# RegulatoryGenomicsGroup/chicdiff

Hardware: NVIDIA B200
Metric: regions tested/sec (agg+NB GLM+dispersion+Wald) (higher is better)
Workload: dtype f64

## Files before the change

chicdiff_b200/csrc/context.cu:

```cuda
#include "../../include/chicdiff_b200.h"
#include "kernels.h"
#include "comm.h"
#include "results_host.h"
#include <algorithm>
#include <climits>
#include <cmath>
#include <cstdarg>
#include <cstdio>
#include <cstdlib>
#include <cstring>
#include <string>
#include <vector>
#include <unistd.h>

using namespace cd;

namespace {

thread_local std::string g_create_error;

template <typename T> struct DevBuf {
    T* p = nullptr;
    size_t cap = 0;
    ~DevBuf() { if (p) cudaFree(p); }
// ... 25 lines not shown
        }
    }
    for (int i = 0; i < p; i++) for (int j = 0; j < p; j++) inv[i * p + j] = a[i][p + j];
    return true;
}

bool build_design(int S, int p, const double* X, CdDesign& d)
{
    memset(&d, 0, sizeof(d));
    d.S = S; d.p = p;
    for (int i = 0; i < S * p; i++) d.X[i] = X[i];
    double xtx[CD_MAXP * CD_MAXP], inv[CD_MAXP * CD_MAXP];
    for (int a = 0; a < p; a++)
        for (int b = 0; b < p; b++) {
            double s = 0;
            for (int j = 0; j < S; j++) s += X[j * p + a] * X[j * p + b];
            xtx[a * p + b] = s;
        }
    if (!invert_small(xtx, p, inv)) return false;
    for (int u = 0; u < p; u++)
        for (int j = 0; j < S; j++) {
            double s = 0;
            for (int v = 0; v < p; v++) s += inv[u * p + v] * X[j * p + v];
            d.ls[u * S + j] = s;
        }
    for (int a = 0; a < S; a++)
        for (int b = 0; b < S; b++) {
            double s = 0;
            for (int u = 0; u < p; u++) s += X[a * p + u] * d.ls[u * S + b];
            d.hat[a * S + b] = s;
        }
    d.ncell = 0;
    for (int j = 0; j < S; j++) {
        int found = -1;
        for (int k = 0; k < j && found < 0; k++) {
            bool same = true;
            for (int u = 0; u < p; u++) if (X[j * p + u] != X[k * p + u]) same = false;
            if (same) found = d.cell[k];
        }
        if (found < 0) { found = d.ncell++; d.cell_size[found] = 0; }
        d.cell[j] = found;
        d.cell_size[found]++;
    }
    d.linear_mu = (d.ncell == p);
    d.any3 = 0;
    for (int c = 0; c < d.ncell; c++) if (d.cell_size[c] >= 3) d.any3 = 1;
    return true;
}

double trigamma_host(double x)
{
    double r = 0.0;
    while (x < 10.0) { r += 1.0 / (x * x); x += 1.0; }
    const double f = 1.0 / (x * x);
    return r + 1.0 / x + 0.5 * f +
           (1.0 / x) * f * (1.0 / 6.0 + f * (-1.0 / 30.0 + f * (1.0 / 42.0 + f * (-1.0 / 30.0 +
           f * (5.0 / 66.0 + f * (-691.0 / 2730.0 + f * (7.0 / 6.0)))))));
}

__global__ void __launch_bounds__(256) dfma_peak_kernel(int iters, double m, double* __restrict__ sink)
{
    double a0 = threadIdx.x, a1 = a0 + 1, a2 = a0 + 2, a3 = a0 + 3, a4 = a0 + 4, a5 = a0 + 5, a6 = a0 + 6, a7 = a0 + 7;
    const double c = 1e-9;
#pragma unroll 16
    for (int k = 0; k < iters; k++) {
        a0 = fma(a0, m, c); a1 = fma(a1, m, c); a2 = fma(a2, m, c); a3 = fma(a3, m, c);
        a4 = fma(a4, m, c); a5 = fma(a5, m, c); a6 = fma(a6, m, c); a7 = fma(a7, m, c);
    }
    const double r = ((a0 + a1) + (a2 + a3)) + ((a4 + a5) + (a6 + a7));
    if (r == 123.456) *sink = r;
}

__global__ void count_evals_kernel(int64_t n, const int32_t* __restrict__ iter, unsigned long long* __restrict__ out)
{
    unsigned long long local = 0;
    for (int64_t i = (int64_t)blockIdx.x * blockDim.x + threadIdx.x; i < n; i += (int64_t)gridDim.x * blockDim.x) {
        const int it = iter[i];
        if (it > 0) local += (unsigned long long)it + 1ull;
    }
    for (int off = 16; off > 0; off >>= 1) local += __shfl_down_sync(0xffffffffu, local, off);
    if ((threadIdx.x & 31) == 0 && local) atomicAdd(out, local);
}

__global__ void count_flags_kernel(int64_t n, const uint8_t* __restrict__ flags, unsigned long long* __restrict__ out)
{
    const int64_t i = (int64_t)blockIdx.x * blockDim.x + threadIdx.x;
    const uint8_t f = (i < n) ? flags[i] : (uint8_t)CD_FLAG_ALLZERO;
    const unsigned nz = __ballot_sync(0xffffffffu, (i < n) && !(f & CD_FLAG_ALLZERO));
    const unsigned gg = __ballot_sync(0xffffffffu, (i < n) && (f & CD_FLAG_GENE_GRID));
    const unsigned mg = __ballot_sync(0xffffffffu, (i < n) && (f & CD_FLAG_MAP_GRID));
    const unsigned bn = __ballot_sync(0xffffffffu, (i < n) && (f & CD_FLAG_BETA_NOCONV));
    if ((threadIdx.x & 31) == 0) {
        if (nz) atomicAdd(out + 0, (unsigned long long)__popc(nz));
        if (gg) atomicAdd(out + 1, (unsigned long long)__popc(gg));
        if (mg) atomicAdd(out + 2, (unsigned long long)__popc(mg));
        if (bn) atomicAdd(out + 3, (unsigned long long)__popc(bn));
    }
}

constexpr int kScalSf = 0;
constexpr int kScalXim = 64;
constexpr int kScalMed = 96;
constexpr int kScalMad = 128;
constexpr int kScalDev = 160;
constexpr int kScalTrend = 192;
constexpr int kScalSums = 384;
constexpr int kScalSize = 1024;
constexpr int kPinTrend = 0, kPinMad = 128, kPinErr = 144, kPinBad = 145, kPinDev = 160, kPinTrendIn = 200, kPinSf = 400;

constexpr int kCntFlags = 0;
constexpr int kCntWait = 4;
constexpr int kCntBad = 7;
constexpr int kCntSelBar = 8;
constexpr int kCntTrendBar = 9;
constexpr int kCntErr = 10;
constexpr int kCntFitDispQueue = 12;
constexpr int kCntPark = 14;
constexpr int kCntWaldQueue = 15;
constexpr int kCntSize = 16;

}

struct cd_ctx {
    int device = 0;
    cudaStream_t st = nullptr;
    std::string err;
    int64_t launches = 0;
    double timings[8] = {0, 0, 0, 0, 0, 0, 0, 0};
    Comm comm;

    bool have_design = false;
    CdDesign des{}, des1{};
    DevBuf<CdDesign> des_dev;
    int64_t n = 0, R = 0;
    bool have_regions = false, have_agg = false, rows_borrowed = false;
    bool have_results = false;
    std::vector<uint8_t> sample_set;
    DevBuf<int64_t> row_off;
    DevBuf<int32_t> N_rows, N_rows_alt;
    DevBuf<double> FM_rows, FM_rows_alt;
    cudaStream_t st_copy = nullptr;
    cudaEvent_t ev_copy = nullptr;
    cudaEvent_t ev_tab_copy = nullptr, ev_tab_used = nullptr;
    bool tab_copy_pending = false;
    cudaEvent_t ev_read[2] = {nullptr, nullptr};
    int front = 0;
    bool front_used = false;
    std::vector<uint8_t> staged;
    int32_t* nbuf(int b) { return b ? N_rows_alt.p : N_rows.p; }
    double* fbuf(int b) { return b ? FM_rows_alt.p : FM_rows.p; }
    int back() const { return front_used ? 1 - front : front; }
    DevBuf<double> BM_rows;
    bool have_bm_rows = false;
    const int32_t* N_rows_p = nullptr;
    const double* FM_rows_p = nullptr;
    DevBuf<int32_t> K;
    DevBuf<double> FM;
    DevBuf<int32_t> Kb;
    int64_t batch_cap = 0;
    DevBuf<double> nf, mu, baseVar, rough, alpha_init, log_alpha, initial_lp, last_lp, dispMAP, dispersion,
        beta, betaSE, stat, pvalue, deviance, maxCooks;
    DevBuf<int32_t> dispGeneIter, dispIter, betaIter, refit_list;
    DevBuf<double> g_baseMean, g_dispGeneEst, g_dispFit, g_resid;
    DevBuf<uint8_t> g_flags;
    DevBuf<double> g_LR;
    DevBuf<unsigned long long> sel_state, sel_hist, sel_aux;
    DevBuf<double> trend_xs;
    DevBuf<double> start_log, log_fit;
    DevBuf<double> partial, scal;
    DevBuf<unsigned long long> counters;
    DevBuf<unsigned long long> eval_counts;
    int n_eval_calls = 0;
    int eval_call_p[16] = {0};
    int64_t eval_call_regions[16] = {0};
    unsigned long long eval_counts_host[16] = {0};
    double trend_passes_batch = 0;
    double trend_passes = 0;
    unsigned long long wait_host[3] = {0, 0, 0};
    DevBuf<int32_t> refit_count;
    DevBuf<int64_t> park_row;
// ... 1241 lines not shown
    CD_CUDA(ctx, ctx->dispGeneIter.ensure(vn)); CD_CUDA(ctx, ctx->dispIter.ensure(vn));
    CD_CUDA(ctx, ctx->betaIter.ensure((size_t)n)); CD_CUDA(ctx, ctx->refit_list.ensure(vn));
    CD_CUDA(ctx, ctx->g_baseMean.ensure(vn)); CD_CUDA(ctx, ctx->g_dispGeneEst.ensure(vn));
    CD_CUDA(ctx, ctx->g_dispFit.ensure(vn)); CD_CUDA(ctx, ctx->g_resid.ensure(vn));
    CD_CUDA(ctx, ctx->g_flags.ensure(vn)); CD_CUDA(ctx, ctx->trend_xs.ensure(vn));
    CD_CUDA(ctx, ctx->start_log.ensure(vn)); CD_CUDA(ctx, ctx->log_fit.ensure(vn));
    CD_CUDA(ctx, ctx->partial.ensure((size_t)kReduceBlocks * kMaxBatch * (CD_MAXS + 1)));
    CD_CUDA(ctx, ctx->scal.ensure(kScalSize));
    if (!ctx->counters.p) {
        CD_CUDA(ctx, ctx->counters.ensure(kCntSize));
        CD_CUDA(ctx, cudaMemsetAsync(ctx->counters.p, 0, kCntSize * sizeof(unsigned long long), st));
    }
    CD_CUDA(ctx, ctx->refit_count.ensure(1));
    CD_CUDA(ctx, ctx->wald_c.ensure((size_t)S * (size_t)n));
    CD_CUDA(ctx, ctx->wald_b0.ensure((size_t)CD_MAXP * (size_t)n));
    CD_CUDA(ctx, ctx->wald_b.ensure((size_t)CD_MAXP * (size_t)n));
    CD_CUDA(ctx, ctx->wald_iter.ensure((size_t)n));
    if (!ctx->lfact.p) {
        CD_CUDA(ctx, ctx->lfact.ensure(kLfactN));
        CD_LAUNCHN(ctx, 1, launch_lfact_table(ctx->lfact.p, st));
    }
    ctx->wald_ws.lfact = ctx->lfact.p;
    ctx->wald_ws.cmat = ctx->wald_c.p; ctx->wald_ws.beta0 = ctx->wald_b0.p; ctx->wald_ws.beta_nat = ctx->wald_b.p;
    ctx->wald_ws.iter = ctx->wald_iter.p; ctx->wald_ws.work_counter = ctx->counters.p + kCntWaldQueue;
    {
        const int64_t cap = nv / 4 + 4096;
        CD_CUDA(ctx, ctx->park_row.ensure((size_t)cap));
        CD_CUDA(ctx, ctx->park_d.ensure((size_t)cap * 5));
        CD_CUDA(ctx, ctx->park_i.ensure((size_t)cap * 2));
        FitDispPark& pk = ctx->park;
        pk.capacity = cap; pk.row = ctx->park_row.p;
        pk.a = ctx->park_d.p; pk.lp = pk.a + cap; pk.dlp = pk.lp + cap; pk.kappa = pk.dlp + cap; pk.lp0 = pk.kappa + cap;
        pk.iter = ctx->park_i.p; pk.iter_accept = pk.iter + cap;
        pk.count = ctx->counters.p + kCntPark;
    }

    CD_CUDA(ctx, ctx->eval_counts.ensure(16));
    CD_CUDA(ctx, cudaMemsetAsync(ctx->eval_counts.p, 0, 16 * sizeof(unsigned long long), st));
    CD_CUDA(ctx, cudaMemsetAsync(ctx->counters.p + kCntWait, 0, 4 * sizeof(unsigned long long), st));
    ctx->n_eval_calls = 0;
    ctx->trend_passes = 0;
    CD_CUDA(ctx, cudaEventRecord(ctx->ev[2], st));
    memset(out->sizeFactors, 0, sizeof(out->sizeFactors));
    for (int k = 2; k < 8; k++) ctx->timings[k] = 0.0;
    ctx->ev_used = 0;
    ctx->tm_begin(6);
    int rc = size_factors(ctx, out->sizeFactors);
    if (rc != CD_OK) return rc;
    ctx->tm_end();

    out->n_deviances = 0;
    BatchOut bo{};
    if (use_grid) {
        rc = run_batch(ctx, ctx->des1, ctx->des_dev.p + 1, ng, CD_NORM_COMBINED, grid, opt->disp_prior_var_grid, grid_len, false, bo, opt);
        if (rc != CD_OK) return rc;
        for (int k = 0; k < ng; k++) {
            out->deviances[k] = bo.sum_deviance[k];
            if (std::isnan(bo.sum_deviance[k]))
                return ctx->fail(CD_ENUMERIC, "theta grid: total deviance is NA (an all-zero region is present and chicdiff.R:1647 "
                                              "sums without na.rm); pass theta explicitly, as chicdiffPipeline does for the control set");
        }
        out->n_deviances = ng;
        int best = -1, nbest = 0;
        for (int k = 0; k < ng; k++) {
            if (best < 0 || out->deviances[k] < out->deviances[best]) { best = k; nbest = 1; }
            else if (out->deviances[k] == out->deviances[best]) nbest++;
        }
        if (nbest != 1) return ctx->fail(CD_ENUMERIC, "theta grid: the minimum total deviance is tied");
        theta = grid[best];
    }
    const double theta_final = std::isnan(theta) ? 0.0 : theta;
    rc = run_batch(ctx, ctx->des, ctx->des_dev.p, 1, norm, &theta_final, opt->disp_prior_var, grid_len, true, bo, opt);
    if (rc != CD_OK) return rc;
    CD_CUDA(ctx, cudaEventRecord(ctx->ev[3], st));
    struct { double a0, a1, varLogDispEsts, dispPriorVar; } po = {bo.a0[0], bo.a1[0], bo.varLogDispEsts[0], bo.dispPriorVar[0]};

    out->theta = (norm == CD_NORM_COMBINED) ? theta : NAN;
    out->trend_a0 = po.a0; out->trend_a1 = po.a1;
    out->varLogDispEsts = po.varLogDispEsts; out->dispPriorVar = po.dispPriorVar;

    CD_CUDA(ctx, cudaMemsetAsync(ctx->counters.p + kCntFlags, 0, 4 * sizeof(unsigned long long), st));
    const uint8_t* flags = ctx->g_flags.p + ctx->g_off;
    if (n > 0) {
        count_flags_kernel<<<(unsigned)((n + 255) / 256), 256, 0, st>>>(n, flags, ctx->counters.p + kCntFlags);
        ctx->launches++;
    }
    unsigned long long hc[4] = {0, 0, 0, 0};
    CD_CUDA(ctx, cudaMemcpyAsync(hc, ctx->counters.p + kCntFlags, sizeof(hc), cudaMemcpyDeviceToHost, st));
    CD_CUDA(ctx, cudaMemcpyAsync(ctx->eval_counts_host, ctx->eval_counts.p, sizeof(ctx->eval_counts_host), cudaMemcpyDeviceToHost, st));
    CD_CUDA(ctx, cudaMemcpyAsync(ctx->wait_host, ctx->counters.p + kCntWait, sizeof(ctx->wait_host), cudaMemcpyDeviceToHost, st));
    const size_t nn = (size_t)n;
    if ((rc = d2h(ctx, out->baseMean, ctx->g_baseMean.p + ctx->g_off, nn)) != CD_OK) return rc;
    if ((rc = d2h(ctx, out->baseVar, ctx->baseVar.p, nn)) != CD_OK) return rc;
    if ((rc = d2h(ctx, out->dispGeneEst, ctx->g_dispGeneEst.p + ctx->g_off, nn)) != CD_OK) return rc;
    if ((rc = d2h(ctx, out->dispFit, ctx->g_dispFit.p + ctx->g_off, nn)) != CD_OK) return rc;
    if ((rc = d2h(ctx, out->dispMAP, ctx->dispMAP.p, nn)) != CD_OK) return rc;
    if ((rc = d2h(ctx, out->dispersion, ctx->dispersion.p, nn)) != CD_OK) return rc;
    if ((rc = d2h(ctx, out->log2FoldChange, ctx->beta.p + (size_t)(p - 1) * nn, nn)) != CD_OK) return rc;
    if ((rc = d2h(ctx, out->lfcSE, ctx->betaSE.p + (size_t)(p - 1) * nn, nn)) != CD_OK) return rc;
    if ((rc = d2h(ctx, out->beta, ctx->beta.p, (size_t)p * nn)) != CD_OK) return rc;
    if ((rc = d2h(ctx, out->betaSE, ctx->betaSE.p, (size_t)p * nn)) != CD_OK) return rc;
    if ((rc = d2h(ctx, out->stat, ctx->stat.p, nn)) != CD_OK) return rc;
    if ((rc = d2h(ctx, out->pvalue, ctx->pvalue.p, nn)) != CD_OK) return rc;
    if ((rc = d2h(ctx, out->deviance, ctx->deviance.p, nn)) != CD_OK) return rc;
    if ((rc = d2h(ctx, out->maxCooks, ctx->maxCooks.p, nn)) != CD_OK) return rc;
    if ((rc = d2h(ctx, out->normFactors, ctx->nf.p, (size_t)S * nn)) != CD_OK) return rc;
    if ((rc = d2h(ctx, out->mu, ctx->mu.p, (size_t)S * nn)) != CD_OK) return rc;
    if ((rc = d2h(ctx, out->dispGeneIter, ctx->dispGeneIter.p, nn)) != CD_OK) return rc;
    if ((rc = d2h(ctx, out->dispIter, ctx->dispIter.p, nn)) != CD_OK) return rc;
    if ((rc = d2h(ctx, out->betaIter, ctx->betaIter.p, nn)) != CD_OK) return rc;
    if ((rc = d2h(ctx, out->flags, flags, nn)) != CD_OK) return rc;
    CD_CUDA(ctx, cudaStreamSynchronize(st));
    out->n_nonzero = (int64_t)hc[0]; out->n_gene_grid = (int64_t)hc[1];
    out->n_map_grid = (int64_t)hc[2]; out->n_beta_noconv = (int64_t)hc[3];
    float ms = 0;
    cudaEventElapsedTime(&ms, ctx->ev[2], ctx->ev[3]);
    ctx->timings[1] = ms;
    ctx->tm_collect();
    ctx->have_results = true;
    return CD_OK;
}

static int results_on_device(cd_ctx* ctx, int64_t n, int S, int p, const double* baseMean, const double* maxCooks,
                             const uint8_t* flags, const double* pvalue, double* pvalue_out, double* padj_out, double* scalars_out)
{
    cudaStream_t st = ctx->st;
    const double alpha = 0.1;
    const double cutoff = res_qf(0.99, (double)p, (double)(S - p));
    const size_t nn = (size_t)std::max<int64_t>(n, 1);
    const int C = res_chunks(n);
    for (int k = 0; k < 4; k++) CD_CUDA(ctx, ctx->res_key[k].ensure(nn));
    for (int k = 0; k < 2; k++) CD_CUDA(ctx, ctx->res_idx[k].ensure(nn));
    CD_CUDA(ctx, ctx->res_pv.ensure(nn)); CD_CUDA(ctx, ctx->res_padj.ensure(nn));
    CD_CUDA(ctx, ctx->res_bms.ensure(nn)); CD_CUDA(ctx, ctx->res_ps.ensure(nn));
    CD_CUDA(ctx, ctx->res_cnt.ensure((size_t)50 * (size_t)std::max(C, 1)));
    CD_CUDA(ctx, ctx->res_cmin.ensure((size_t)std::max(C, 1))); CD_CUDA(ctx, ctx->res_smin.ensure((size_t)std::max(C, 1)));
    CD_CUDA(ctx, ctx->res_small.ensure(2 + 50 + 50));
    CD_CUDA(ctx, ctx->res_smalld.ensure(100));
    unsigned long long* counts = ctx->res_small.p;
    unsigned long long* m_tot = ctx->res_small.p + 2;
    unsigned long long* best = ctx->res_small.p + 52;
    double* cut = ctx->res_smalld.p;
    double* theta = ctx->res_smalld.p + 50;
    unsigned long long *pkey0 = ctx->res_key[0].p, *pkey1 = ctx->res_key[1].p, *bmkey0 = ctx->res_key[2].p, *bmkey1 = ctx->res_key[3].p;
    unsigned int *idx0 = ctx->res_idx[0].p, *idx1 = ctx->res_idx[1].p;

    CD_LAUNCHN(ctx, 1, res_launch_keys(n, p, cutoff, baseMean, maxCooks, flags, pvalue, ctx->res_pv.p, ctx->res_padj.p,
                                       pkey0, bmkey0, idx0, counts, st));
    int j = 0;
    double cut_h[50], theta_h[50];
    for (int k = 0; k < 50; k++) { cut_h[k] = NAN; theta_h[k] = (k == 49) ? .95 : 0.0 + k * ((.95 - 0.0) / 49); }
    if (n > 0) {
        size_t bytes = 0;
        CD_CUDA(ctx, cp_sort_pairs_u64(nullptr, bytes, bmkey0, bmkey1, idx0, idx1, n, st));
        CD_CUDA(ctx, ctx->res_tmp.ensure(bytes));
        CD_LAUNCHN(ctx, 1, cp_sort_pairs_u64(ctx->res_tmp.p, bytes, bmkey0, bmkey1, idx0, idx1, n, st));
        CD_LAUNCHN(ctx, 1, res_launch_cutoffs(n, bmkey1, counts, cut, theta, st));
        CD_LAUNCHN(ctx, 1, cp_sort_pairs_u64(ctx->res_tmp.p, bytes, pkey0, pkey1, idx0, idx1, n, st));
        CD_LAUNCHN(ctx, 1, res_launch_gather(n, idx1, baseMean, ctx->res_pv.p, ctx->res_bms.p, ctx->res_ps.p, st));
        CD_LAUNCHN(ctx, 3, res_launch_num_rej(n, counts, ctx->res_bms.p, ctx->res_ps.p, cut, ctx->res_cnt.p, m_tot, alpha, best, st));
        unsigned long long best_h[50];
        CD_CUDA(ctx, cudaMemcpyAsync(best_h, best, sizeof(best_h), cudaMemcpyDeviceToHost, st));
        CD_CUDA(ctx, cudaMemcpyAsync(cut_h, cut, sizeof(cut_h), cudaMemcpyDeviceToHost, st));
        CD_CUDA(ctx, cudaMemcpyAsync(theta_h, theta, sizeof(theta_h), cudaMemcpyDeviceToHost, st));
        CD_CUDA(ctx, cudaStreamSynchronize(st));
        double numRej[50];
        for (int k = 0; k < 50; k++) numRej[k] = (double)best_h[k];
// ... 169 lines not shown
```

chicdiff_b200/csrc/dispersion.cu:

```cuda
#include "kernels.h"
#include <cuda_pipeline.h>
#include "posterior.cuh"

namespace cd {

static inline int blocks_for(int64_t n, int threads) { return (int)((n + threads - 1) / threads); }

__global__ void __launch_bounds__(256)
norm_factors_kernel(int64_t n, int S, int G, const double* __restrict__ FMagg, const double* __restrict__ sf,
                    int mode, BatchScalars theta, double* __restrict__ nf, const int32_t* __restrict__ K,
                    int32_t* __restrict__ Kb)
{
    const int64_t i = (int64_t)blockIdx.x * blockDim.x + threadIdx.x;
    if (i >= n) return;
    const int64_t nv = (int64_t)G * n;
    if (Kb) {
        for (int s = 0; s < S; s++) {
            const int32_t k = K[(int64_t)s * n + i];
            for (int g = 0; g < G; g++) Kb[(int64_t)s * nv + (int64_t)g * n + i] = k;
        }
    }
    if (mode == 0) {
        for (int s = 0; s < S; s++)
            for (int g = 0; g < G; g++) nf[(int64_t)s * nv + (int64_t)g * n + i] = sf[s];
        return;
    }
    double acc = 0.0;
    for (int s = 0; s < S; s++) acc += log(FMagg[(int64_t)s * n + i]);
    const double gm = exp(acc / S);
    double m3[CD_MAXS];
    bool anyna = false;
    for (int s = 0; s < S; s++) {
        m3[s] = FMagg[(int64_t)s * n + i] / gm;
        anyna = anyna || isnan(m3[s]);
    }
    if (anyna)
        for (int s = 0; s < S; s++) m3[s] = sf[s];
    if (mode == 1) {
        for (int s = 0; s < S; s++)
            for (int g = 0; g < G; g++) nf[(int64_t)s * nv + (int64_t)g * n + i] = m3[s];
        return;
    }
    for (int g = 0; g < G; g++) {
        const double th = theta.v[g];
        double acc2 = 0.0;
        for (int s = 0; s < S; s++) acc2 += log(m3[s] * (1.0 - th) + sf[s] * th);
        const double g2 = exp(acc2 / S);
        for (int s = 0; s < S; s++)
            nf[(int64_t)s * nv + (int64_t)g * n + i] = (m3[s] * (1.0 - th) + sf[s] * th) / g2;
    }
}

cudaError_t launch_norm_factors(int64_t n, int S, int G, const double* FMagg, const double* sf, int mode,
                                const BatchScalars& theta, double* nf, const int32_t* K, int32_t* Kb, cudaStream_t st)
{
    if (n == 0) return cudaSuccess;
    norm_factors_kernel<<<blocks_for(n, 256), 256, 0, st>>>(n, S, G, FMagg, sf, mode, theta, nf, K, Kb);
    return cudaGetLastError();
}

__global__ void __launch_bounds__(256)
base_stats_kernel(int64_t n, int S, const CdDesign* __restrict__ des, const int32_t* __restrict__ K,
                  const double* __restrict__ nf, double* __restrict__ baseMean, double* __restrict__ baseVar,
                  double* __restrict__ rough, uint8_t* __restrict__ flags, double* __restrict__ mu)
{
    __shared__ double hat[CD_MAXS * CD_MAXS];
    for (int k = threadIdx.x; k < S * S; k += blockDim.x) hat[k] = des->hat[k];
    __syncthreads();
    const int p = des->p;
    const int64_t i = (int64_t)blockIdx.x * blockDim.x + threadIdx.x;
    if (i >= n) return;
    double q[CD_MAXS];
    double sum = 0.0;
    int64_t tot = 0;
    for (int j = 0; j < S; j++) {
        const int32_t k = K[(int64_t)j * n + i];
        q[j] = (double)k / nf[(int64_t)j * n + i];
        sum += q[j];
        tot += k;
    }
    const double m = sum / S;
    double v = 0.0;
    for (int j = 0; j < S; j++) v += (q[j] - m) * (q[j] - m);
    baseMean[i] = m;
    baseVar[i] = v / (S - 1);
    flags[i] = (tot == 0) ? CD_FLAG_ALLZERO : 0;
    double est = 0.0;
    for (int a = 0; a < S; a++) {
        double mul = 0.0;
        for (int b = 0; b < S; b++) mul += hat[a * S + b] * q[b];
        const double mm = fmax(1.0, mul);
        est += ((q[a] - mm) * (q[a] - mm) - mm) / (mm * mm);
        if (mu) mu[(int64_t)a * n + i] = (tot == 0) ? NAN : fmax(mul * nf[(int64_t)a * n + i], kMinMu);
    }
    rough[i] = fmax(est / (S - p), 0.0);
}

cudaError_t launch_base_stats(int64_t n, int S, const CdDesign* des, const int32_t* K, const double* nf, double* baseMean,
                              double* baseVar, double* rough, uint8_t* flags, double* mu, cudaStream_t st)
{
    if (n == 0) return cudaSuccess;
    base_stats_kernel<<<blocks_for(n, 256), 256, 0, st>>>(n, S, des, K, nf, baseMean, baseVar, rough, flags, mu);
    return cudaGetLastError();
}

__global__ void __launch_bounds__(256)
gene_init_kernel(int64_t n, int64_t n_fit, int S, const double* __restrict__ baseMean, const double* __restrict__ baseVar,
                 const double* __restrict__ rough, const uint8_t* __restrict__ flags,
                 const double* __restrict__ xim_dev, double* __restrict__ alpha_init, double* __restrict__ start_log)
{
    const int64_t i = (int64_t)blockIdx.x * blockDim.x + threadIdx.x;
    if (i >= n) return;
    if (flags[i] & CD_FLAG_ALLZERO) {
        alpha_init[i] = NAN;
        start_log[i] = NAN;
        return;
    }
    const double xim = xim_dev[i / n_fit];
    const double bm = baseMean[i], bv = baseVar[i];
    const double moments = (bv - xim * bm) / (bm * bm);
    const double maxDisp = fmax(10.0, (double)S);
    const double a0 = fmin(fmax(kMinDisp, fmin(rough[i], moments)), maxDisp);
    alpha_init[i] = a0;
    start_log[i] = log_pos(a0);
}

cudaError_t launch_gene_init(int64_t n, int64_t n_fit, int S, const double* baseMean, const double* baseVar,
                             const double* rough, const uint8_t* flags, const double* xim_dev, double* alpha_init,
                             double* start_log, cudaStream_t st)
{
    if (n == 0) return cudaSuccess;
    gene_init_kernel<<<blocks_for(n, 256), 256, 0, st>>>(n, n_fit, S, baseMean, baseVar, rough, flags, xim_dev, alpha_init,
                                                       start_log);
    return cudaGetLastError();
}

constexpr int kFitDispThreads = 128;
constexpr int kFitDispTripCap = 24;

__host__ __device__ static inline size_t fit_disp_block_doubles(int S) { return (size_t)16 * S + (size_t)32 * S + 64; }

static inline size_t fit_disp_smem_doubles(int S, int P, int threads)
{
    return (size_t)2 * S * threads + (size_t)(threads / 32) * 2 * fit_disp_block_doubles(S) + (size_t)S * P;
}

constexpr double kSearchEpsilon = 1.0e-4, kSearchKappa0 = 1.0, kSearchTol = 1e-6;
constexpr int kSearchMaxit = 100;

struct SearchState {
    double a, lp, lp0, dlp, kappa;
    int iter, iter_accept;
};

__device__ __forceinline__ double propose(SearchState& s)
{
    s.iter++;
    const double a_propose = s.a + s.kappa * s.dlp;
    if (a_propose < -30.0) s.kappa = (-30.0 - s.a) / s.dlp;
    if (a_propose > 10.0) s.kappa = (10.0 - s.a) / s.dlp;
    return s.a + s.kappa * s.dlp;
}

__device__ __forceinline__ bool decide(SearchState& s, double x, double lpx, double dlpx, double min_log_alpha)
{
    bool finished = false;
    const double theta_kappa = -1.0 * lpx;
    const double theta_hat_kappa = -1.0 * s.lp - s.kappa * kSearchEpsilon * (s.dlp * s.dlp);
    if (theta_kappa <= theta_hat_kappa) {
        s.iter_accept++;
        s.a = x;
        const double change = lpx - s.lp;
        if (change < kSearchTol) { s.lp = lpx; finished = true; }
        else if (s.a < min_log_alpha) { finished = true; }
        else {
            s.lp = lpx;
            s.dlp = dlpx;
            s.kappa = fmin(s.kappa * 1.1, kSearchKappa0);
            if (s.iter_accept % 5 == 0) s.kappa = s.kappa / 2.0;
        }
    } else {
        s.kappa = s.kappa / 2.0;
    }
    if (s.iter >= kSearchMaxit) finished = true;
    return finished;
// ... 274 lines not shown
            double tr = 0.0;
#pragma unroll
            for (int u = 0; u < P; u++)
#pragma unroll
                for (int v = 0; v < P; v++) tr += Bi.v[sidx<P>(u, v)] * dB.v[sidx<P>(v, u)];
            double lpx = red[2 * NS] + cr;
            double dlpx = ((r * r) * red[2 * NS + 1] - 0.5 * tr) * alpha;
            if (use_prior) {
                const double d = x - prior_mean;
                lpx += -0.5 * d * d / prior_sigmasq;
                dlpx += -1.0 * d / prior_sigmasq;
            }
            if (active && decide(s, x, lpx, dlpx, min_log_alpha)) {
                if (lane_g == 0) { log_alpha_out[i] = s.a; iter_out[i] = s.iter; initial_lp_out[i] = s.lp0; last_lp_out[i] = s.lp; }
                active = false;
            }
        }
    }
}

template <int P>
static cudaError_t launch_fit_disp_p(int64_t n, int64_t n_fit, int S, const CdDesign* des, const int32_t* K, const double* mu,
                                     const double* start_log, const double* prior_log_mean, const BatchScalars& prior_sigmasq,
                                     double* log_alpha, int32_t* iter, double* initial_lp, double* last_lp,
                                     unsigned long long* work_counter, const FitDispPark& park, cudaStream_t st)
{
    const int threads = kFitDispThreads;
    const int64_t want = (n + threads - 1) / threads;
    const size_t smem = fit_disp_smem_doubles(S, P, threads) * sizeof(double);
    int dev = 0, sms = 148;
    cudaGetDevice(&dev);
    cudaDeviceGetAttribute(&sms, cudaDevAttrMultiProcessorCount, dev);
    const int G = S <= 8 ? 8 : (S <= 16 ? 16 : 32);
    const bool tile = (double)n * 0.04 * G <= (double)sms * 1024.0;
    BatchScalars prior_inv;
    for (int g = 0; g < kMaxBatch; g++) prior_inv.v[g] = 1.0 / prior_sigmasq.v[g];
    int per_sm = 1;
    cudaError_t e = cudaFuncSetAttribute(fit_disp_kernel<P, false>, cudaFuncAttributeMaxDynamicSharedMemorySize, (int)smem);
    if (e != cudaSuccess) return e;
    e = cudaOccupancyMaxActiveBlocksPerMultiprocessor(&per_sm, fit_disp_kernel<P, false>, threads, smem);
    if (e != cudaSuccess) return e;
    const int64_t resident = (int64_t)sms * (per_sm > 0 ? per_sm : 1);
    const int blocks = (int)(want < resident ? want : resident);
    fit_disp_kernel<P, false><<<blocks, threads, smem, st>>>(n, n_fit, S, des, K, mu, start_log, prior_log_mean, prior_inv,
                                                             log_alpha, iter, initial_lp, last_lp, work_counter, park);
    if (tile) {
        auto* tile_kernel = G == 8 ? fit_disp_resume_tile_kernel<P, 8>
                                   : (G == 16 ? fit_disp_resume_tile_kernel<P, 16> : fit_disp_resume_tile_kernel<P, 32>);
        tile_kernel<<<sms * 8, 128, 0, st>>>(n, n_fit, S, des, K, mu, prior_log_mean, prior_sigmasq, log_alpha, iter,
                                             initial_lp, last_lp, park);
    } else {
        e = cudaFuncSetAttribute(fit_disp_kernel<P, true>, cudaFuncAttributeMaxDynamicSharedMemorySize, (int)smem);
        if (e != cudaSuccess) return e;
        const int64_t want2 = (park.capacity + threads - 1) / threads;
        const int blocks2 = (int)(want2 < resident ? want2 : resident);
        fit_disp_kernel<P, true><<<blocks2 > 0 ? blocks2 : 1, threads, smem, st>>>(n, n_fit, S, des, K, mu, start_log,
            prior_log_mean, prior_inv, log_alpha, iter, initial_lp, last_lp, work_counter + 1, park);
    }
    return cudaGetLastError();
}

cudaError_t launch_fit_disp(int64_t n, int64_t n_fit, int S, int p, const CdDesign* des, const int32_t* K, const double* mu,
                            const double* start_log, const double* prior_log_mean, const BatchScalars& prior_sigmasq,
                            double* log_alpha, int32_t* iter, double* initial_lp, double* last_lp,
                            unsigned long long* work_counter, const FitDispPark& park, cudaStream_t st)
{
    if (n == 0) return cudaSuccess;
    cudaError_t e = cudaMemsetAsync(work_counter, 0, 2 * sizeof(unsigned long long), st);
    if (e != cudaSuccess) return e;
    e = cudaMemsetAsync(park.count, 0, sizeof(unsigned long long), st);
    if (e != cudaSuccess) return e;
    decltype(&launch_fit_disp_p<1>) launch;
    switch (p) {
        case 1: launch = launch_fit_disp_p<1>; break;
        case 2: launch = launch_fit_disp_p<2>; break;
        case 3: launch = launch_fit_disp_p<3>; break;
        case 4: launch = launch_fit_disp_p<4>; break;
        default: return cudaErrorInvalidValue;
    }
    return launch(n, n_fit, S, des, K, mu, start_log, prior_log_mean, prior_sigmasq, log_alpha, iter, initial_lp, last_lp,
                  work_counter, park, st);
}

__global__ void __launch_bounds__(256)
gene_post_kernel(int64_t n, int S, const double* __restrict__ alpha_init, const double* __restrict__ log_alpha,
                 const int32_t* __restrict__ iter, const double* __restrict__ initial_lp,
                 const double* __restrict__ last_lp, uint8_t* __restrict__ flags,
                 double* __restrict__ dispGeneEst, int32_t* __restrict__ refit_list,
                 int32_t* __restrict__ refit_count)
{
    const int64_t i = (int64_t)blockIdx.x * blockDim.x + threadIdx.x;
    if (i >= n) return;
    uint8_t f = flags[i];
    if (f & CD_FLAG_ALLZERO) { dispGeneEst[i] = NAN; return; }
    const double maxDisp = fmax(10.0, (double)S);
    double disp = fmin(exp(log_alpha[i]), maxDisp);
    const double l0 = initial_lp[i];
    if (last_lp[i] < l0 + fabs(l0) / 1e6) { disp = alpha_init[i]; f |= CD_FLAG_GENE_NOINCREASE; }
    const int it = iter[i];
    const bool conv = (it < kSearchMaxit) && (it != 1);
    if (!conv && disp > kMinDisp * 10.0) {
        f |= CD_FLAG_GENE_GRID;
        const int32_t slot = atomicAdd(refit_count, 1);
        refit_list[slot] = (int32_t)i;
    }
    dispGeneEst[i] = fmin(fmax(disp, kMinDisp), maxDisp);
    flags[i] = f;
}

cudaError_t launch_gene_post(int64_t n, int S, const double* alpha_init, const double* log_alpha, const int32_t* iter,
                             const double* initial_lp, const double* last_lp, uint8_t* flags, double* dispGeneEst,
                             int32_t* refit_list, int32_t* refit_count, cudaStream_t st)
{
    cudaError_t e = cudaMemsetAsync(refit_count, 0, sizeof(int32_t), st);
    if (e != cudaSuccess || n == 0) return e;
    gene_post_kernel<<<blocks_for(n, 256), 256, 0, st>>>(n, S, alpha_init, log_alpha, iter, initial_lp, last_lp,
                                                       flags, dispGeneEst, refit_list, refit_count);
    return cudaGetLastError();
}

__global__ void __launch_bounds__(256)
map_post_kernel(int64_t n, int64_t n_fit, int S, const double* __restrict__ log_alpha, const int32_t* __restrict__ iter,
                const double* __restrict__ dispGeneEst, const double* __restrict__ dispFit, BatchScalars outlier_thr,
                uint8_t* __restrict__ flags, double* __restrict__ dispMAP, double* __restrict__ dispersion,
                int32_t* __restrict__ refit_list, int32_t* __restrict__ refit_count)
{
    const int64_t i = (int64_t)blockIdx.x * blockDim.x + threadIdx.x;
    if (i >= n) return;
    uint8_t f = flags[i];
    if (f & CD_FLAG_ALLZERO) { dispMAP[i] = NAN; dispersion[i] = NAN; return; }
    const double maxDisp = fmax(10.0, (double)S);
    if (!(iter[i] < kSearchMaxit)) {
        f |= CD_FLAG_MAP_GRID;
        const int32_t slot = atomicAdd(refit_count, 1);
        refit_list[slot] = (int32_t)i;
    }
    const double dmap = fmin(fmax(exp(log_alpha[i]), kMinDisp), maxDisp);
    const double ge = dispGeneEst[i], ft = dispFit[i];
    const bool outl = log(ge) > log(ft) + outlier_thr.v[(int)(i / n_fit)];
    if (outl) f |= CD_FLAG_OUTLIER;
    dispMAP[i] = dmap;
    dispersion[i] = outl ? ge : dmap;
    flags[i] = f;
}

cudaError_t launch_map_post(int64_t n, int64_t n_fit, int S, const double* log_alpha, const int32_t* iter,
                            const double* dispGeneEst, const double* dispFit, const BatchScalars& outlier_thr, uint8_t* flags,
                            double* dispMAP, double* dispersion, int32_t* refit_list, int32_t* refit_count, cudaStream_t st)
{
    cudaError_t e = cudaMemsetAsync(refit_count, 0, sizeof(int32_t), st);
    if (e != cudaSuccess || n == 0) return e;
    map_post_kernel<<<blocks_for(n, 256), 256, 0, st>>>(n, n_fit, S, log_alpha, iter, dispGeneEst, dispFit, outlier_thr,
                                                      flags, dispMAP, dispersion, refit_list, refit_count);
    return cudaGetLastError();
}

template <int P>
__global__ void __launch_bounds__(128)
fit_disp_grid_kernel(int64_t n, int64_t n_fit, int S, const CdDesign* __restrict__ des, const int32_t* __restrict__ n_list_dev,
                     const int32_t* __restrict__ list, const int32_t* __restrict__ K, const double* __restrict__ mu_g,
                     const double* __restrict__ prior_mean_disp, BatchScalars prior_sigmasq_g, int grid_len,
                     double* __restrict__ disp_out, double* __restrict__ dispersion_out,
                     const uint8_t* __restrict__ flags, const double* __restrict__ dispGeneEst)
{
    __shared__ double sh[4][2 * CD_MAXS];
    __shared__ double Xs[CD_MAXS * CD_MAXP];
    for (int k = threadIdx.x; k < S * P; k += blockDim.x) Xs[k] = des->X[k];
    __syncthreads();
    const LogTab tab = 0;
    const int lane = threadIdx.x & 31;
    const int wib = threadIdx.x >> 5;
    const int warps_per_block = blockDim.x >> 5;
    const int n_list = *n_list_dev;
    double* ys = sh[wib];
    double* mus = sh[wib] + CD_MAXS;
    for (int w = blockIdx.x * warps_per_block + wib; w < n_list; w += gridDim.x * warps_per_block) {
        const int64_t i = list[w];
        __syncwarp();
        if (lane < S) {
            ys[lane] = (double)K[(int64_t)lane * n + i];
            mus[lane] = mu_g[(int64_t)lane * n + i];
        }
        __syncwarp();
        const bool use_prior = (prior_mean_disp != nullptr);
        const double prior_mean = use_prior ? log(prior_mean_disp[i]) : 0.0;
        const double prior_sigmasq = 1.0 / prior_sigmasq_g.v[(int)(i / n_fit)];
        const double maxDisp = fmax(10.0, (double)S);
        const double lo = log(1e-8), hi = log(maxDisp);
        const double step = (hi - lo) / (grid_len - 1);
        double best_a = lo;
        double from = lo, to = hi, by = step;
        for (int level = 0; level < 2; level++) {
            const double a = (lane == grid_len - 1) ? to : from + lane * by;
            double v = -INFINITY, unused;
            if (lane < grid_len) eval_post<P, false, false>(a, ys, mus, 1, S, Xs, tab, prior_mean, prior_sigmasq, use_prior, v, unused);
            int idx = lane;
#pragma unroll
            for (int off = 16; off > 0; off >>= 1) {
                const double ov = __shfl_xor_sync(0xffffffffu, v, off);
                const int oi = __shfl_xor_sync(0xffffffffu, idx, off);
                if (ov > v || (ov == v && oi < idx)) { v = ov; idx = oi; }
            }
            best_a = (idx == grid_len - 1) ? to : from + idx * by;
            if (level == 0) {
                const double delta = (lo + step) - lo;
                from = best_a - delta;
                to = best_a + delta;
                by = (to - from) / (grid_len - 1);
            }
        }
        if (lane == 0) {
            const double d = fmin(fmax(exp(best_a), kMinDisp), maxDisp);
            disp_out[i] = d;
            if (dispersion_out) dispersion_out[i] = (flags[i] & CD_FLAG_OUTLIER) ? dispGeneEst[i] : d;
        }
    }
}

cudaError_t launch_fit_disp_grid(int64_t n, int64_t n_fit, int S, int p, const CdDesign* des, const int32_t* n_list_dev,
                                 const int32_t* list, const int32_t* K, const double* mu, const double* prior_mean_disp,
                                 const BatchScalars& prior_sigmasq, int grid_len, double* disp_out, double* dispersion_out,
                                 const uint8_t* flags, const double* dispGeneEst, cudaStream_t st)
// ... 21 lines not shown
```

chicdiff_b200/csrc/offsets.cu:

```cuda
#include "kernels.h"

namespace cd {

static inline int blocks_for(int64_t n, int threads) { return (int)((n + threads - 1) / threads); }

constexpr long long kSpinLimit = 20000000000LL;

template <int NV>
__device__ __forceinline__ void block_reduce_store(double (&v)[NV], double* dst)
{
    __shared__ double sh[NV][8];
    const int lane = threadIdx.x & 31, wid = threadIdx.x >> 5;
#pragma unroll
    for (int k = 0; k < NV; k++) {
        double x = v[k];
#pragma unroll
        for (int off = 16; off > 0; off >>= 1) x += __shfl_down_sync(0xffffffffu, x, off);
        if (lane == 0) sh[k][wid] = x;
    }
    __syncthreads();
    if (threadIdx.x < NV) {
        double x = 0.0;
        const int nw = blockDim.x >> 5;
        for (int w = 0; w < nw; w++) x += sh[threadIdx.x][w];
        dst[threadIdx.x] = x;
    }
    __syncthreads();
}

__global__ void __launch_bounds__(32) final_reduce_kernel(int nblocks, int nv, const double* __restrict__ partial,
                                                          double* __restrict__ out)
{
    const int k = blockIdx.x;
    double x = 0.0;
    for (int b = threadIdx.x; b < nblocks; b += 32) x += partial[(size_t)b * nv + k];
#pragma unroll
    for (int off = 16; off > 0; off >>= 1) x += __shfl_down_sync(0xffffffffu, x, off);
    if (threadIdx.x == 0) out[k] = x;
}

__global__ void __launch_bounds__(256)
masked_colsums_kernel(int64_t n, int G, int S, const double* __restrict__ M, const uint8_t* __restrict__ mask,
                      double* __restrict__ partial)
{
    const int64_t nv = (int64_t)G * n;
    const int64_t chunk = (n + gridDim.x - 1) / gridDim.x;
    const int64_t lo = (int64_t)blockIdx.x * chunk;
    const int64_t hi = (lo + chunk < n) ? lo + chunk : n;
    for (int g = 0; g < G; g++)
        for (int s = 0; s <= S; s++) {
            double v[1] = {0.0};
            for (int64_t i = lo + threadIdx.x; i < hi; i += blockDim.x) {
                const int64_t r = (int64_t)g * n + i;
                const bool use = (mask == nullptr) || ((mask[r] & CD_FLAG_ALLZERO) == 0);
                if (use) v[0] += (s < S) ? M[(int64_t)s * nv + r] : 1.0;
            }
            block_reduce_store<1>(v, partial + ((size_t)blockIdx.x * G + g) * (S + 1) + s);
        }
}

cudaError_t launch_masked_colsums(int64_t n, int G, int S, const double* M, const uint8_t* mask, double* partial,
                                  double* out, cudaStream_t st)
{
    masked_colsums_kernel<<<kReduceBlocks, 256, 0, st>>>(n, G, S, M, mask, partial);
    final_reduce_kernel<<<G * (S + 1), 32, 0, st>>>(kReduceBlocks, G * (S + 1), partial, out);
    return cudaGetLastError();
}

__global__ void __launch_bounds__(256)
segment_sums_kernel(int64_t n, int G, const double* __restrict__ v_in, double* __restrict__ partial)
{
    const int64_t chunk = (n + gridDim.x - 1) / gridDim.x;
    const int64_t lo = (int64_t)blockIdx.x * chunk;
    const int64_t hi = (lo + chunk < n) ? lo + chunk : n;
    for (int g = 0; g < G; g++) {
        double v[1] = {0.0};
        for (int64_t i = lo + threadIdx.x; i < hi; i += blockDim.x) v[0] += v_in[(int64_t)g * n + i];
        block_reduce_store<1>(v, partial + (size_t)blockIdx.x * G + g);
    }
}

cudaError_t launch_segment_sums(int64_t n, int G, const double* v, double* partial, double* out, cudaStream_t st)
{
    segment_sums_kernel<<<kReduceBlocks, 256, 0, st>>>(n, G, v, partial);
    final_reduce_kernel<<<G, 32, 0, st>>>(kReduceBlocks, G, partial, out);
    return cudaGetLastError();
}

__global__ void xim_kernel(int G, int S, const double* __restrict__ sums, double* __restrict__ xim)
{
    const int g = threadIdx.x;
    if (g >= G) return;
    const double* sg = sums + (size_t)g * (S + 1);
    const double cnt = sg[S];
    double acc = 0.0;
    for (int s = 0; s < S; s++) acc += 1.0 / (sg[s] / cnt);
    xim[g] = acc / S;
}

cudaError_t launch_xim(int G, int S, const double* sums, double* xim, cudaStream_t st)
{
    xim_kernel<<<1, 32, 0, st>>>(G, S, sums, xim);
    return cudaGetLastError();
}

__global__ void __launch_bounds__(256)
log_ratios_kernel(int64_t n, int S, const int32_t* __restrict__ K, double* __restrict__ LR, double* __restrict__ bad)
{
    const int64_t i = (int64_t)blockIdx.x * blockDim.x + threadIdx.x;
    if (i >= n) return;
    double acc = 0.0;
    bool ok = true, neg = false;
    for (int s = 0; s < S; s++) {
        const int32_t k = K[(int64_t)s * n + i];
        ok = ok && (k > 0);
        neg = neg || (k < 0);
        acc += log((double)k);
    }
    if (neg) *bad = 1.0;
    const double lgm = acc / S;
    for (int s = 0; s < S; s++)
        LR[(int64_t)s * n + i] = ok ? log((double)K[(int64_t)s * n + i]) - lgm : INFINITY;
}

cudaError_t launch_log_ratios(int64_t n, int S, const int32_t* K, double* LR, double* bad, cudaStream_t st)
{
    if (n == 0) return cudaSuccess;
    log_ratios_kernel<<<blocks_for(n, 256), 256, 0, st>>>(n, S, K, LR, bad);
    return cudaGetLastError();
}

constexpr int kTrendThreads = 512;
constexpr int kTrendSlot = 8 * kMaxBatch + 8;

__device__ __forceinline__ bool trend_grid_barrier(unsigned int* bar, unsigned int nblocks, unsigned int& phase,
                                                   unsigned long long* err)
{
    __shared__ int ok_sh;
    __syncthreads();
    phase++;
    if (threadIdx.x == 0) {
        __threadfence();
        atomicAdd(bar, 1u);
        int ok = 1;
        const long long t0 = clock64();
        while (atomicAdd(bar, 0u) < phase * nblocks) {
            if (*reinterpret_cast<volatile unsigned long long*>(err) != 0ull) { ok = 0; break; }
// ... 311 lines not shown
```

Measured before the change: 84.77 million.

## Fuse colsum passes, template sample count, aggregate atomics in flag and refit kernels

The masked column-sum kernel now accumulates all S+1 sums in one pass over rows instead of re-reading the mask and data for each sample. Base stats and colsums are templated on a maximum sample count so per-row arrays can live in registers. Flag counting becomes grid-stride with shared-memory aggregation, refit-list appends use warp-aggregated atomics, and outlier thresholds are staged in shared memory. These target repeated memory passes, atomic contention and local-memory spills, at the cost of more template instantiations and higher register pressure for large S.

New measurement: 86.29 million, median of 6. +1.8%, better.

```diff
diff --git a/chicdiff_b200/csrc/context.cu b/chicdiff_b200/csrc/context.cu
--- a/chicdiff_b200/csrc/context.cu
+++ b/chicdiff_b200/csrc/context.cu
@@ -131,20 +131,27 @@
     if ((threadIdx.x & 31) == 0 && local) atomicAdd(out, local);
 }
 
-__global__ void count_flags_kernel(int64_t n, const uint8_t* __restrict__ flags, unsigned long long* __restrict__ out)
-{
-    const int64_t i = (int64_t)blockIdx.x * blockDim.x + threadIdx.x;
-    const uint8_t f = (i < n) ? flags[i] : (uint8_t)CD_FLAG_ALLZERO;
-    const unsigned nz = __ballot_sync(0xffffffffu, (i < n) && !(f & CD_FLAG_ALLZERO));
-    const unsigned gg = __ballot_sync(0xffffffffu, (i < n) && (f & CD_FLAG_GENE_GRID));
-    const unsigned mg = __ballot_sync(0xffffffffu, (i < n) && (f & CD_FLAG_MAP_GRID));
-    const unsigned bn = __ballot_sync(0xffffffffu, (i < n) && (f & CD_FLAG_BETA_NOCONV));
-    if ((threadIdx.x & 31) == 0) {
-        if (nz) atomicAdd(out + 0, (unsigned long long)__popc(nz));
-        if (gg) atomicAdd(out + 1, (unsigned long long)__popc(gg));
-        if (mg) atomicAdd(out + 2, (unsigned long long)__popc(mg));
-        if (bn) atomicAdd(out + 3, (unsigned long long)__popc(bn));
-    }
+__global__ void __launch_bounds__(256) count_flags_kernel(int64_t n, const uint8_t* __restrict__ flags,
+                                                          unsigned long long* __restrict__ out)
+{
+    __shared__ unsigned int cnt[4];
+    if (threadIdx.x < 4) cnt[threadIdx.x] = 0u;
+    __syncthreads();
+    unsigned int c[4] = {0u, 0u, 0u, 0u};
+    const int64_t stride = (int64_t)gridDim.x * blockDim.x;
+    for (int64_t base = (int64_t)blockIdx.x * blockDim.x; base < n; base += stride) {
+        const int64_t i = base + threadIdx.x;
+        const uint8_t f = (i < n) ? flags[i] : (uint8_t)CD_FLAG_ALLZERO;
+        c[0] += __popc(__ballot_sync(0xffffffffu, (i < n) && !(f & CD_FLAG_ALLZERO)));
+        c[1] += __popc(__ballot_sync(0xffffffffu, (i < n) && (f & CD_FLAG_GENE_GRID)));
+        c[2] += __popc(__ballot_sync(0xffffffffu, (i < n) && (f & CD_FLAG_MAP_GRID)));
+        c[3] += __popc(__ballot_sync(0xffffffffu, (i < n) && (f & CD_FLAG_BETA_NOCONV)));
+    }
+    if ((threadIdx.x & 31) == 0)
+        for (int k = 0; k < 4; k++)
+            if (c[k]) atomicAdd(&cnt[k], c[k]);
+    __syncthreads();
+    if (threadIdx.x < 4 && cnt[threadIdx.x]) atomicAdd(out + threadIdx.x, (unsigned long long)cnt[threadIdx.x]);
 }
 
 constexpr int kScalSf = 0;
@@ -1552,7 +1559,8 @@
     CD_CUDA(ctx, cudaMemsetAsync(ctx->counters.p + kCntFlags, 0, 4 * sizeof(unsigned long long), st));
     const uint8_t* flags = ctx->g_flags.p + ctx->g_off;
     if (n > 0) {
-        count_flags_kernel<<<(unsigned)((n + 255) / 256), 256, 0, st>>>(n, flags, ctx->counters.p + kCntFlags);
+        const unsigned nb = (unsigned)std::min<int64_t>((n + 255) / 256, kReduceBlocks);
+        count_flags_kernel<<<nb, 256, 0, st>>>(n, flags, ctx->counters.p + kCntFlags);
         ctx->launches++;
     }
     unsigned long long hc[4] = {0, 0, 0, 0};
diff --git a/chicdiff_b200/csrc/dispersion.cu b/chicdiff_b200/csrc/dispersion.cu
--- a/chicdiff_b200/csrc/dispersion.cu
+++ b/chicdiff_b200/csrc/dispersion.cu
@@ -59,39 +59,51 @@
     return cudaGetLastError();
 }
 
+template <int SMAX>
 __global__ void __launch_bounds__(256)
 base_stats_kernel(int64_t n, int S, const CdDesign* __restrict__ des, const int32_t* __restrict__ K,
                   const double* __restrict__ nf, double* __restrict__ baseMean, double* __restrict__ baseVar,
                   double* __restrict__ rough, uint8_t* __restrict__ flags, double* __restrict__ mu)
 {
-    __shared__ double hat[CD_MAXS * CD_MAXS];
+    __shared__ double hat[SMAX * SMAX];
     for (int k = threadIdx.x; k < S * S; k += blockDim.x) hat[k] = des->hat[k];
     __syncthreads();
     const int p = des->p;
     const int64_t i = (int64_t)blockIdx.x * blockDim.x + threadIdx.x;
     if (i >= n) return;
-    double q[CD_MAXS];
+    double q[SMAX];
     double sum = 0.0;
     int64_t tot = 0;
-    for (int j = 0; j < S; j++) {
-        const int32_t k = K[(int64_t)j * n + i];
-        q[j] = (double)k / nf[(int64_t)j * n + i];
-        sum += q[j];
-        tot += k;
+#pragma unroll
+    for (int j = 0; j < SMAX; j++) {
+        q[j] = 0.0;
+        if (j < S) {
+            const int32_t k = K[(int64_t)j * n + i];
+            q[j] = (double)k / nf[(int64_t)j * n + i];
+            sum += q[j];
+            tot += k;
+        }
     }
     const double m = sum / S;
     double v = 0.0;
-    for (int j = 0; j < S; j++) v += (q[j] - m) * (q[j] - m);
+#pragma unroll
+    for (int j = 0; j < SMAX; j++)
+        if (j < S) v += (q[j] - m) * (q[j] - m);
     baseMean[i] = m;
     baseVar[i] = v / (S - 1);
     flags[i] = (tot == 0) ? CD_FLAG_ALLZERO : 0;
     double est = 0.0;
-    for (int a = 0; a < S; a++) {
-        double mul = 0.0;
-        for (int b = 0; b < S; b++) mul += hat[a * S + b] * q[b];
-        const double mm = fmax(1.0, mul);
-        est += ((q[a] - mm) * (q[a] - mm) - mm) / (mm * mm);
-        if (mu) mu[(int64_t)a * n + i] = (tot == 0) ? NAN : fmax(mul * nf[(int64_t)a * n + i], kMinMu);
+#pragma unroll
+    for (int a = 0; a < SMAX; a++) {
+        if (a < S) {
+            double mul = 0.0;
+#pragma unroll
+            for (int b = 0; b < SMAX; b++)
+                if (b < S) mul += hat[a * S + b] * q[b];
+            const double mm = fmax(1.0, mul);
+            est += ((q[a] - mm) * (q[a] - mm) - mm) / (mm * mm);
+            if (mu) mu[(int64_t)a * n + i] = (tot == 0) ? NAN : fmax(mul * nf[(int64_t)a * n + i], kMinMu);
+        }
     }
     rough[i] = fmax(est / (S - p), 0.0);
 }
@@ -100,7 +112,10 @@
                               double* baseVar, double* rough, uint8_t* flags, double* mu, cudaStream_t st)
 {
     if (n == 0) return cudaSuccess;
-    base_stats_kernel<<<blocks_for(n, 256), 256, 0, st>>>(n, S, des, K, nf, baseMean, baseVar, rough, flags, mu);
+    const int nb = blocks_for(n, 256);
+    if (S <= 8) base_stats_kernel<8><<<nb, 256, 0, st>>>(n, S, des, K, nf, baseMean, baseVar, rough, flags, mu);
+    else if (S <= 16) base_stats_kernel<16><<<nb, 256, 0, st>>>(n, S, des, K, nf, baseMean, baseVar, rough, flags, mu);
+    else base_stats_kernel<CD_MAXS><<<nb, 256, 0, st>>>(n, S, des, K, nf, baseMean, baseVar, rough, flags, mu);
     return cudaGetLastError();
 }
 
@@ -541,6 +556,18 @@
                   work_counter, park, st);
 }
 
+__device__ __forceinline__ void append_refit_row(int32_t* __restrict__ refit_list, int32_t* __restrict__ refit_count,
+                                                 int32_t row)
+{
+    const unsigned active = __activemask();
+    const unsigned lane = threadIdx.x & 31u;
+    const int leader = __ffs(active) - 1;
+    int32_t base = 0;
+    if ((int)lane == leader) base = atomicAdd(refit_count, __popc(active));
+    base = __shfl_sync(active, base, leader);
+    refit_list[base + __popc(active & ((1u << lane) - 1u))] = row;
+}
+
 __global__ void __launch_bounds__(256)
 gene_post_kernel(int64_t n, int S, const double* __restrict__ alpha_init, const double* __restrict__ log_alpha,
                  const int32_t* __restrict__ iter, const double* __restrict__ initial_lp,
@@ -560,8 +587,7 @@
     const bool conv = (it < kSearchMaxit) && (it != 1);
     if (!conv && disp > kMinDisp * 10.0) {
         f |= CD_FLAG_GENE_GRID;
-        const int32_t slot = atomicAdd(refit_count, 1);
-        refit_list[slot] = (int32_t)i;
+        append_refit_row(refit_list, refit_count, (int32_t)i);
     }
     dispGeneEst[i] = fmin(fmax(disp, kMinDisp), maxDisp);
     flags[i] = f;
@@ -584,6 +610,12 @@
                 uint8_t* __restrict__ flags, double* __restrict__ dispMAP, double* __restrict__ dispersion,
                 int32_t* __restrict__ refit_list, int32_t* __restrict__ refit_count)
 {
+    __shared__ double thr[kMaxBatch];
+    if (threadIdx.x == 0) {
+#pragma unroll
+        for (int g = 0; g < kMaxBatch; g++) thr[g] = outlier_thr.v[g];
+    }
+    __syncthreads();
     const int64_t i = (int64_t)blockIdx.x * blockDim.x + threadIdx.x;
     if (i >= n) return;
     uint8_t f = flags[i];
@@ -591,12 +623,11 @@
     const double maxDisp = fmax(10.0, (double)S);
     if (!(iter[i] < kSearchMaxit)) {
         f |= CD_FLAG_MAP_GRID;
-        const int32_t slot = atomicAdd(refit_count, 1);
-        refit_list[slot] = (int32_t)i;
+        append_refit_row(refit_list, refit_count, (int32_t)i);
     }
     const double dmap = fmin(fmax(exp(log_alpha[i]), kMinDisp), maxDisp);
     const double ge = dispGeneEst[i], ft = dispFit[i];
-    const bool outl = log(ge) > log(ft) + outlier_thr.v[(int)(i / n_fit)];
+    const bool outl = log(ge) > log(ft) + thr[(int)(i / n_fit)];
     if (outl) f |= CD_FLAG_OUTLIER;
     dispMAP[i] = dmap;
     dispersion[i] = outl ? ge : dmap;
diff --git a/chicdiff_b200/csrc/offsets.cu b/chicdiff_b200/csrc/offsets.cu
--- a/chicdiff_b200/csrc/offsets.cu
+++ b/chicdiff_b200/csrc/offsets.cu
@@ -39,30 +39,58 @@
     if (threadIdx.x == 0) out[k] = x;
 }
 
+template <int SMAX>
 __global__ void __launch_bounds__(256)
 masked_colsums_kernel(int64_t n, int G, int S, const double* __restrict__ M, const uint8_t* __restrict__ mask,
                       double* __restrict__ partial)
 {
+    __shared__ double sh[SMAX + 1][8];
+    const int lane = threadIdx.x & 31, wid = threadIdx.x >> 5;
     const int64_t nv = (int64_t)G * n;
     const int64_t chunk = (n + gridDim.x - 1) / gridDim.x;
     const int64_t lo = (int64_t)blockIdx.x * chunk;
     const int64_t hi = (lo + chunk < n) ? lo + chunk : n;
-    for (int g = 0; g < G; g++)
-        for (int s = 0; s <= S; s++) {
-            double v[1] = {0.0};
-            for (int64_t i = lo + threadIdx.x; i < hi; i += blockDim.x) {
-                const int64_t r = (int64_t)g * n + i;
-                const bool use = (mask == nullptr) || ((mask[r] & CD_FLAG_ALLZERO) == 0);
-                if (use) v[0] += (s < S) ? M[(int64_t)s * nv + r] : 1.0;
-            }
-            block_reduce_store<1>(v, partial + ((size_t)blockIdx.x * G + g) * (S + 1) + s);
-        }
+    for (int g = 0; g < G; g++) {
+        double v[SMAX + 1];
+#pragma unroll
+        for (int s = 0; s <= SMAX; s++) v[s] = 0.0;
+        for (int64_t i = lo + threadIdx.x; i < hi; i += blockDim.x) {
+            const int64_t r = (int64_t)g * n + i;
+            const bool use = (mask == nullptr) || ((mask[r] & CD_FLAG_ALLZERO) == 0);
+            if (use) {
+#pragma unroll
+                for (int s = 0; s < SMAX; s++)
+                    if (s < S) v[s] += M[(int64_t)s * nv + r];
+                v[SMAX] += 1.0;
+            }
+        }
+#pragma unroll
+        for (int s = 0; s <= SMAX; s++) {
+            if (s < S || s == SMAX) {
+                double x = v[s];
+#pragma unroll
+                for (int off = 16; off > 0; off >>= 1) x += __shfl_down_sync(0xffffffffu, x, off);
+                if (lane == 0) sh[s][wid] = x;
+            }
+        }
+        __syncthreads();
+        if ((int)threadIdx.x <= S) {
+            const int s = ((int)threadIdx.x < S) ? (int)threadIdx.x : SMAX;
+            double x = 0.0;
+            const int nw = blockDim.x >> 5;
+            for (int w = 0; w < nw; w++) x += sh[s][w];
+            partial[((size_t)blockIdx.x * G + g) * (S + 1) + threadIdx.x] = x;
+        }
+        __syncthreads();
+    }
 }
 
 cudaError_t launch_masked_colsums(int64_t n, int G, int S, const double* M, const uint8_t* mask, double* partial,
                                   double* out, cudaStream_t st)
 {
-    masked_colsums_kernel<<<kReduceBlocks, 256, 0, st>>>(n, G, S, M, mask, partial);
+    if (S <= 8) masked_colsums_kernel<8><<<kReduceBlocks, 256, 0, st>>>(n, G, S, M, mask, partial);
+    else if (S <= 16) masked_colsums_kernel<16><<<kReduceBlocks, 256, 0, st>>>(n, G, S, M, mask, partial);
+    else masked_colsums_kernel<CD_MAXS><<<kReduceBlocks, 256, 0, st>>>(n, G, S, M, mask, partial);
     final_reduce_kernel<<<G * (S + 1), 32, 0, st>>>(kReduceBlocks, G * (S + 1), partial, out);
     return cudaGetLastError();
 }
```
